# PinataFarms/DAD-3DHeads

Measured on AMD Instinct MI355X. Metric: images/sec (FLAME decode + 445-lmk projection), batch 64 @ 256^2, higher is better.
Workload: dtype f32

## Files before the change

### dad-3dheads_amd/csrc/capi.cpp

```cpp
#include <algorithm>
#include <cmath>
#include <cstdlib>
#include <cstring>
#include <memory>
#include <mutex>

#include "common.hpp"

namespace dad3d {

static thread_local std::string g_last_error;

void set_error(const char* fmt, ...) {
    char buf[1024];
    va_list ap;
    va_start(ap, fmt);
    vsnprintf(buf, sizeof buf, fmt, ap);
    va_end(ap);
    g_last_error = buf;
}

template <typename T>
static dad3d_status upload(T** dst, const std::vector<T>& src) {
    *dst = nullptr;
    const size_t bytes = std::max<size_t>(src.size(), 1) * sizeof(T);
    DAD3D_HIP_TRY(hipMalloc(reinterpret_cast<void**>(dst), bytes));
    if (!src.empty()) DAD3D_HIP_TRY(hipMemcpy(*dst, src.data(), src.size() * sizeof(T), hipMemcpyHostToDevice));
    return DAD3D_OK;
}

}

using namespace dad3d;

static void free_device(int device, std::initializer_list<void*> ptrs) {
    DeviceGuard guard(device);
    for (void* p : ptrs) (void)hipFree(p);
}

struct FlameConsts {
    int device = 0;
    float *d_bpack = nullptr, *d_jdirs = nullptr, *d_j0 = nullptr, *d_w8 = nullptr;
    float* d_bpack_pipe = nullptr;
    float split_b_scale = 1.0f;
    float* d_bpack_f16 = nullptr;
    std::mutex f16_mu;
    int n_tiles_pipe = 0;
    float* d_gpack = nullptr;
    std::mutex gpack_mutex;
    ~FlameConsts() { free_device(device, {d_bpack, d_jdirs, d_j0, d_w8, d_gpack, d_bpack_pipe, d_bpack_f16}); }
};

struct LandmarkList {
    int device = 0;
    int n = 0;
    int *d_head = nullptr, *d_next = nullptr;
    float4* d_vtab = nullptr;
    std::unique_ptr<FlameConsts> sub;
    int sub_verts = 0;
    float4* d_sub_vtab = nullptr;
    ~LandmarkList() { free_device(device, {d_head, d_next, d_vtab, d_sub_vtab}); }
};

struct FlameShape {
    int device = 0;
    int n_verts = 0, n_betas = 0;
    ParamLayout lay{};
    int parents[kNumJoints]{};
    int n_pose_feats = 0, pose_feat_first = 0;
    int kgroups = 0, ksteps = 0;
    int n_tiles = 0, n_tiles_pad8 = 0;
    int max_shape = 300;
    float image_size = 256.f;
};

struct dad3d_flame : FlameShape {
    std::shared_ptr<FlameConsts> c;
    std::shared_ptr<LandmarkList> lmk;
    int kernel_choice = -1;
    float* d_bwd_partials = nullptr;
    int bwd_cap = 0;
    float* d_grad_partials = nullptr;
    size_t grad_cap = 0;
    float* d_imgc = nullptr;
    unsigned* d_sync = nullptr;
    unsigned arrive_total = 0;
    int cap_nbb = 0;
    bool profiling = false;
    unsigned long long* d_trace = nullptr;
    uint64_t trace_capacity = 0;
    char* d_split_a = nullptr;
    int split_cap = 0;
    std::vector<char*> split_retired;
    hipEvent_t ev_first = nullptr, ev_last = nullptr;
    int prof_launches = 0;
    ~dad3d_flame() {
        DeviceGuard guard(device);
        for (void* p : {(void*)d_sync, (void*)d_imgc, (void*)d_bwd_partials, (void*)d_grad_partials, (void*)d_split_a}) (void)hipFree(p);
        for (char* p : split_retired) (void)hipFree(p);
        if (ev_first) (void)hipEventDestroy(ev_first);
        if (ev_last) (void)hipEventDestroy(ev_last);
    }
};

static int decode_kernel_choice() {
    static const int choice = [] {
        const char* e = getenv("DAD3D_DECODE_KERNEL");
        if (!e) return 0;
        if (e[0] == 'v' && e[1] == '1') return DAD3D_KERNEL_TWO_ROLE;
        if (std::strcmp(e, "split") == 0) return DAD3D_KERNEL_SPLIT_BF16;
        if (std::strcmp(e, "split_f16") == 0) return DAD3D_KERNEL_SPLIT_F16;
        return std::strcmp(e, "force_pipe") == 0 ? DAD3D_KERNEL_PIPELINED : DAD3D_KERNEL_AUTO;
    }();
    return choice;
}

static size_t frag_offset(int tile, int kgroups, int g, int col, int q) {
    return ((((size_t)tile * kgroups + g) * 4 + col / 16) * 64 + (col % 16) + 16 * q) * 4;
}
template <typename F>
static void for_each_fragment(std::vector<float>& pack, int n_tiles, int kgroups, F&& f) {
    for (int t = 0; t < n_tiles; ++t)
        for (int g = 0; g < kgroups; ++g)
            for (int col = 0; col < kTileCols; ++col)
                for (int q = 0; q < 4; ++q) f(t, g, col, q, &pack[frag_offset(t, kgroups, g, col, q)]);
}

static int grad_chunks(const dad3d_flame* h) { return (h->n_verts * 3 + kGradChunk - 1) / kGradChunk; }

static dad3d_status grad_inputs_prepare(dad3d_flame* h, int batch, hipStream_t s) {
    const int pad = (batch + kBlockImages - 1) / kBlockImages * kBlockImages;
    const int per_slice = grad_chunks_per_slice(pad);
    const size_t rows = (size_t)((grad_chunks(h) + per_slice - 1) / per_slice) * pad;
    bool need_pack;
    {
        std::lock_guard<std::mutex> lock(h->c->gpack_mutex);
        need_pack = h->c->d_gpack == nullptr;
    }
    const bool need_scratch = rows > h->grad_cap;
    if (!need_pack && !need_scratch) return DAD3D_OK;
    hipStreamCaptureStatus capture = hipStreamCaptureStatusNone;
    if (s != nullptr) (void)hipStreamIsCapturing(s, &capture);
    DAD3D_REQUIRE(capture == hipStreamCaptureStatusNone,
                  "the first training step of a handle (and the first at a larger batch) allocates: run it once before capturing a graph");
    DAD3D_REQUIRE(h->n_betas + 36 <= kGradRows, "dad3d_flame_grad_inputs: %d inputs exceed %d", h->n_betas + 36, kGradRows);
    if (need_pack) {
        std::lock_guard<std::mutex> lock(h->c->gpack_mutex);
        if (!h->c->d_gpack) {
            float* pack = nullptr;
            DAD3D_HIP_TRY(hipMalloc(reinterpret_cast<void**>(&pack), grad_pack_floats(grad_chunks(h)) * sizeof(float)));
            GradPackArgs pa{h->c->d_bpack, pack, h->kgroups, h->n_betas, h->n_pose_feats, h->pose_feat_first, h->n_betas + 36,
                            h->n_verts * 3, grad_chunks(h)};
            dad3d_status st = launch_grad_pack(pa, nullptr);
            if (st == DAD3D_OK && hipDeviceSynchronize() != hipSuccess) st = DAD3D_E_HIP;
            if (st) {
                (void)hipFree(pack);
                set_error("building the basis^T pack failed");
                return st;
            }
            h->c->d_gpack = pack;
        }
    }
    if (need_scratch) {
        DAD3D_HIP_TRY(hipDeviceSynchronize());
        (void)hipFree(h->d_grad_partials);
        h->d_grad_partials = nullptr;
        h->grad_cap = 0;
        DAD3D_HIP_TRY(hipMalloc(reinterpret_cast<void**>(&h->d_grad_partials), rows * kGradRows * sizeof(float)));
        h->grad_cap = rows;
    }
    return DAD3D_OK;
}

static dad3d_status flame_reserve(dad3d_flame* h, int nbb) {
    if (nbb <= h->cap_nbb) return DAD3D_OK;
    if (h->d_imgc) (void)hipFree(h->d_imgc);
    h->d_imgc = nullptr;
    h->cap_nbb = 0;
    DAD3D_HIP_TRY(hipMalloc(reinterpret_cast<void**>(&h->d_imgc), (size_t)nbb * kBlockImages * kImgConsts * sizeof(float)));
    h->cap_nbb = nbb;
    return DAD3D_OK;
}

static bool landmark_subset_enabled() {
    static const bool on = [] {
        const char* e = getenv("DAD3D_LANDMARK_SUBSET");
        return !(e && e[0] == '0');
    }();
    return on;
}

static dad3d_status build_landmark_sub(const dad3d_flame* h, const int64_t* idx, int n, const std::vector<float4>& vtab, LandmarkList* L) {
    std::vector<char> named(h->n_verts, 0);
    for (int s = 0; s < n; ++s) named[idx[s]] = 1;
    std::vector<int> uniq;
    for (int v = 0; v < h->n_verts; ++v)
        if (named[v]) uniq.push_back(v);
    const int nu = (int)uniq.size(), nt = (nu + kPipeTileVerts - 1) / kPipeTileVerts;
    if ((size_t)nu * 3 > (size_t)h->n_verts) return DAD3D_OK;
    std::vector<float> full((size_t)h->c->n_tiles_pipe * kPipeKGroups * 4 * 64 * 4), pack((size_t)nt * kPipeKGroups * 4 * 64 * 4, 0.0f);
    DAD3D_HIP_TRY(hipMemcpy(full.data(), h->c->d_bpack_pipe, full.size() * sizeof(float), hipMemcpyDeviceToHost));
    for_each_fragment(pack, nt, kPipeKGroups, [&](int t, int g, int col, int q, float* dst) {
        int src_tile = 0, src_col = col;
        if (col < 3 * kPipeTileVerts) {
            const int u = t * kPipeTileVerts + col / 3;
            if (u >= nu) return;
            src_tile = uniq[u] / kPipeTileVerts, src_col = (uniq[u] % kPipeTileVerts) * 3 + col % 3;
        }
        std::copy_n(&full[frag_offset(src_tile, kPipeKGroups, g, src_col, q)], 4, dst);
    });
    std::vector<float4> sub_vtab(nu);
    for (int u = 0; u < nu; ++u) sub_vtab[u] = vtab[uniq[u]];
    L->sub.reset(new FlameConsts);
    L->sub->device = h->device;
    L->sub->n_tiles_pipe = nt;
    L->sub->split_b_scale = h->c->split_b_scale;
    L->sub_verts = nu;
    const dad3d_status st = upload(&L->sub->d_bpack_pipe, pack);
    return st ? st : upload(&L->d_sub_vtab, sub_vtab);
}

static dad3d_status build_landmarks(const dad3d_flame* h, const int64_t* idx, int n, std::shared_ptr<LandmarkList>* out) {
    const int V = h->n_verts;
    std::vector<int> head(V, -1), next(n, -1);
    for (int s = n - 1; s >= 0; --s) {
        next[s] = head[idx[s]];
        head[idx[s]] = s;
    }
    std::vector<int> head2((size_t)V * 2, -1);
    for (int v = 0; v < V; ++v)
        if (head[v] >= 0) head2[(size_t)v * 2] = head[v], head2[(size_t)v * 2 + 1] = next[head[v]];
    auto L = std::make_shared<LandmarkList>();
    L->device = h->device;
    L->n = n;
    dad3d_status st;
    if ((st = upload(&L->d_head, head2)) || (st = upload(&L->d_next, next))) return st;
    if (h->c->d_bpack_pipe) {
        std::vector<float> w8((size_t)V * 8);
        DAD3D_HIP_TRY(hipMemcpy(w8.data(), h->c->d_w8, w8.size() * sizeof(float), hipMemcpyDeviceToHost));
        std::vector<float4> vtab(V);
        for (int v = 0; v < V; ++v) {
            const float* w = &w8[(size_t)v * 8];
            float fh, fn;
            memcpy(&fh, &head2[(size_t)v * 2], 4), memcpy(&fn, &head2[(size_t)v * 2 + 1], 4);
            vtab[v] = float4{w[5] + w[2], w[2], fh, fn};
        }
        if ((st = upload(&L->d_vtab, vtab))) return st;
        if (landmark_subset_enabled() && n > 0 && (st = build_landmark_sub(h, idx, n, vtab, L.get()))) return st;
    }
    *out = std::move(L);
    return DAD3D_OK;
}

extern "C" {

const char* dad3d_last_error(void) { return g_last_error.c_str(); }
void dad3d_clear_error(void) { g_last_error.clear(); }
int dad3d_version(void) { return DAD3D_VERSION; }
const char* dad3d_build_info(void) {
    static const std::string info = [] {
        int rt = 0, drv = 0;
        (void)hipRuntimeGetVersion(&rt);
        (void)hipDriverGetVersion(&drv);
        char buf[384];
        snprintf(buf, sizeof buf, "built: clang %s, HIP headers %d.%d.%d; running: HIP runtime %d, driver %d", __clang_version__, HIP_VERSION_MAJOR,
                 HIP_VERSION_MINOR, HIP_VERSION_PATCH, rt, drv);
        return std::string(buf);
// ... 153 lines not shown
    h->lmk = parent->lmk;
    h->kernel_choice = parent->kernel_choice;
    dad3d_status st;
    if ((st = upload(&h->d_sync, std::vector<unsigned>(kSyncWords, 0u))) || (st = flame_reserve(h.get(), 1))) return st;
    *out = h.release();
    return DAD3D_OK;
}

int dad3d_flame_num_params(const dad3d_flame* h) { return h ? h->lay.n_params : -1; }
int dad3d_flame_num_verts(const dad3d_flame* h) { return h ? h->n_verts : -1; }
int dad3d_flame_num_landmarks(const dad3d_flame* h) { return h ? h->lmk->n : -1; }
int dad3d_flame_num_landmark_vertices(const dad3d_flame* h) { return h ? h->lmk->sub_verts : 0; }

dad3d_status dad3d_flame_set_landmarks(dad3d_flame* h, const int64_t* idx, int n) {
    DAD3D_REQUIRE(h && n >= 0 && (idx || n == 0), "dad3d_flame_set_landmarks: bad argument");
    for (int s = 0; s < n; ++s)
        DAD3D_REQUIRE(idx[s] >= 0 && idx[s] < h->n_verts, "landmark index %lld out of range [0,%d)", (long long)idx[s], h->n_verts);
    DeviceGuard guard(h->device);
    std::shared_ptr<LandmarkList> list;
    dad3d_status st = build_landmarks(h, idx, n, &list);
    if (st) return st;
    DAD3D_HIP_TRY(hipDeviceSynchronize());
    h->lmk = std::move(list);
    return DAD3D_OK;
}

static uint64_t trace_entries_two_role(const dad3d_flame* h, int batch) {
    const uint64_t nbb = (batch + kBlockImages - 1) / kBlockImages, pose_blocks = ((uint64_t)(batch + 3) / 4 + 7) / 8 * 8;
    return ((uint64_t)h->n_tiles_pad8 * nbb * 8 + pose_blocks * 4) * 32;
}
static uint64_t trace_entries_pipe(const dad3d_flame* h) { return (uint64_t)h->c->n_tiles_pipe * 8 * 32; }

static dad3d_status ensure_basis_f16(FlameConsts* c, hipStream_t s) {
    std::lock_guard<std::mutex> lock(c->f16_mu);
    if (c->d_bpack_f16) return DAD3D_OK;
    hipStreamCaptureStatus capture = hipStreamCaptureStatusNone;
    if (s != nullptr) (void)hipStreamIsCapturing(s, &capture);
    DAD3D_REQUIRE(capture == hipStreamCaptureStatusNone, "the first fp16-split decode of a model builds its basis planes: run it once before capturing a graph");
    const size_t bytes = (size_t)c->n_tiles_pipe * kPipeKGroups * 4 * 64 * 4 * sizeof(float);
    float* d = nullptr;
    DAD3D_HIP_TRY(hipMalloc(reinterpret_cast<void**>(&d), bytes));
    dad3d_status st = launch_split_basis_f16(c->d_bpack_pipe, d, c->n_tiles_pipe, c->split_b_scale, s);
    if (st == DAD3D_OK && hipStreamSynchronize(s) != hipSuccess) {
        set_error("ensure_basis_f16: hipStreamSynchronize failed");
        st = DAD3D_E_HIP;
    }
    if (st) {
        (void)hipFree(d);
        return st;
    }
    c->d_bpack_f16 = d;
    return DAD3D_OK;
}

static dad3d_status ensure_split_scratch(dad3d_flame* h, int n_phase, hipStream_t s) {
    if (n_phase <= h->split_cap) return DAD3D_OK;
    hipStreamCaptureStatus capture = hipStreamCaptureStatusNone;
    if (s != nullptr) (void)hipStreamIsCapturing(s, &capture);
    DAD3D_REQUIRE(capture == hipStreamCaptureStatusNone,
                  "the first split-kernel decode of a handle (and the first at a larger batch) allocates: run it once before capturing a graph");
    if (h->d_split_a) h->split_retired.push_back(h->d_split_a);
    h->d_split_a = nullptr, h->split_cap = 0;
    DAD3D_HIP_TRY(hipMalloc(reinterpret_cast<void**>(&h->d_split_a), (size_t)n_phase * kSplitBlockBytes));
    DAD3D_HIP_TRY(hipMemsetAsync(h->d_split_a, 0, (size_t)n_phase * kSplitBlockBytes, s));
    h->split_cap = n_phase;
    return DAD3D_OK;
}

static int resolve_kernel(const dad3d_flame* h, int pinned, int batch, unsigned flags, bool posed) {
    const bool pipe_covers = h->c->d_bpack_pipe && !posed && !(flags & (DAD3D_COMPAT_CROSS_B3 | DAD3D_ZERO_ROTATION)) &&
                             (size_t)batch * h->n_verts * 12 < ((size_t)1 << 31) && (size_t)batch * std::max(h->lmk->n, 1) * 8 < ((size_t)1 << 31);
    if (pinned == DAD3D_KERNEL_TWO_ROLE || (pinned == DAD3D_KERNEL_AUTO && !pipe_covers)) return DAD3D_KERNEL_TWO_ROLE;
    if (pipe_covers) return pinned == DAD3D_KERNEL_AUTO ? DAD3D_KERNEL_PIPELINED : pinned;
    set_error("dad3d_flame_decode: the %s kernel does not cover this launch (model, flags or output size)",
              pinned == DAD3D_KERNEL_PIPELINED ? "pipelined" : "split");
    return -1;
}

static dad3d_status decode_impl(dad3d_flame* h, float* params, int batch, unsigned flags, float* verts3d, float* proj,
                                float* lmk_xy, int32_t* lmk_px, float* posed, void* stream) {
    DAD3D_REQUIRE(h, "dad3d_flame_decode: null handle");
    DAD3D_REQUIRE(batch >= 0, "dad3d_flame_decode: negative batch");
    if (batch == 0) return DAD3D_OK;
    DAD3D_REQUIRE(params, "dad3d_flame_decode: null params");
    DAD3D_REQUIRE(!((flags & DAD3D_FLIP_Z) && (flags & DAD3D_TO_2D)), "DAD3D_FLIP_Z needs a 3-component projection");
    DAD3D_REQUIRE(!(posed && (flags & DAD3D_COMPAT_CROSS_B3)), "DAD3D_COMPAT_CROSS_B3 is inference-only (dad3d_flame_decode_posed refuses it)");
    DeviceGuard guard(h->device);
    hipStream_t s = static_cast<hipStream_t>(stream);
    const int pinned = h->kernel_choice >= 0 ? h->kernel_choice : decode_kernel_choice();
    const int kernel = resolve_kernel(h, pinned, batch, flags, posed != nullptr);
    if (kernel < 0) return DAD3D_E_UNSUPPORTED;
    const LandmarkList& L = *h->lmk;
    const int n_lmk = (lmk_xy || lmk_px) ? L.n : 0;

    const bool on_sub = L.sub && !verts3d && !proj && n_lmk && !h->d_trace && pinned != DAD3D_KERNEL_PIPELINED;
    FlameConsts* c = on_sub ? L.sub.get() : h->c.get();
    const float4* vtab = on_sub ? L.d_sub_vtab : L.d_vtab;
    const int n_verts = on_sub ? L.sub_verts : h->n_verts;

    dad3d_status st;
    if (kernel == DAD3D_KERNEL_SPLIT_BF16 || kernel == DAD3D_KERNEL_SPLIT_F16) {
        DAD3D_REQUIRE(!h->d_trace, "dad3d_flame_decode: the split kernels have no trace stamps");
        const int n_phase = (batch + kSplitRows - 1) / kSplitRows;
        st = ensure_split_scratch(h, n_phase, s);
        if (!st && kernel == DAD3D_KERNEL_SPLIT_F16) st = ensure_basis_f16(c, s);
        if (!st && kernel == DAD3D_KERNEL_SPLIT_F16 && L.sub) st = ensure_basis_f16(L.sub.get(), s);
        if (st) return st;
        SplitArgs sa{};
        sa.params = params;
        sa.bpack = c->d_bpack_pipe;
        sa.bpack_f16 = c->d_bpack_f16;
        sa.vtab = vtab;
        sa.lmk_next = L.d_next;
        sa.verts3d = verts3d;
        sa.proj = proj;
        sa.lmk_xy = lmk_xy;
        sa.lmk_px = lmk_px;
        sa.aplanes = h->d_split_a;
        sa.b_scale = c->split_b_scale;
        sa.n_params = h->lay.n_params;
        sa.batch = batch;
        sa.n_phase = n_phase;
        sa.n_tiles = c->n_tiles_pipe;
        split_chunking(sa.n_tiles, n_phase, &sa.n_chunks, &sa.phases_per_chunk);
        sa.n_verts = n_verts;
        sa.n_lmk = n_lmk;
        sa.image_size = h->image_size;
        sa.flags = flags & 0xFFu;
        st = launch_flame_decode_split(sa, kernel, s);
    } else if (kernel == DAD3D_KERNEL_PIPELINED) {
        DAD3D_REQUIRE(!h->d_trace || h->trace_capacity >= trace_entries_pipe(h), "dad3d_flame_decode: the trace buffer holds %llu entries, "
                      "this launch stamps %llu (dad3d_flame_debug_trace_entries)", (unsigned long long)h->trace_capacity,
                      (unsigned long long)trace_entries_pipe(h));
        PipeArgs pa{};
        pa.params = params;
        pa.bpack = c->d_bpack_pipe;
        pa.vtab = vtab;
        pa.lmk_next = L.d_next;
        pa.verts3d = verts3d;
        pa.proj = proj;
        pa.lmk_xy = lmk_xy;
        pa.lmk_px = lmk_px;
        pa.trace = h->d_trace;
        pa.n_params = h->lay.n_params;
        pa.batch = batch;
        pa.n_half = (batch + kPipeHalf - 1) / kPipeHalf;
        pa.n_tiles = c->n_tiles_pipe;
        pa.n_verts = n_verts;
        pa.n_lmk = n_lmk;
        pa.image_size = h->image_size;
        pa.flags = flags & 0xFFu;
        pa.n_chunks = 1;
        if (!h->d_trace && (!proj || (flags & DAD3D_TO_2D))) pipe_chunking(pa.n_tiles, pa.n_half, &pa.chunk_half, &pa.n_chunks, &pa.wg_per_xcd);
        st = launch_flame_decode_pipe(pa, s);
    } else {
        DAD3D_REQUIRE(!h->d_trace || h->trace_capacity >= trace_entries_two_role(h, batch), "dad3d_flame_decode: the trace buffer holds %llu "
                      "entries, this launch stamps %llu (dad3d_flame_debug_trace_entries)", (unsigned long long)h->trace_capacity,
                      (unsigned long long)trace_entries_two_role(h, batch));
        if (posed && batch <= DAD3D_GRAD_INPUTS_MAX_BATCH && h->n_betas + 36 <= kGradRows && (st = grad_inputs_prepare(h, batch, s))) return st;
        const int nbb = (batch + kBlockImages - 1) / kBlockImages;
        if (nbb > h->cap_nbb) {
            DAD3D_HIP_TRY(hipDeviceSynchronize());
            if ((st = flame_reserve(h, nbb))) return st;
        }
        DecodeArgs da{};
        da.params = params;
        da.bpack = h->c->d_bpack;
        da.jdirs = h->c->d_jdirs;
        da.j0 = h->c->d_j0;
        da.weights8 = h->c->d_w8;
        da.lmk_head = L.d_head;
        da.lmk_next = L.d_next;
        da.imgc = h->d_imgc;
        da.sync = h->d_sync;
        da.verts3d = verts3d;
        da.proj = proj;
        da.lmk_xy = lmk_xy;
        da.lmk_px = lmk_px;
        da.posed = posed;
        da.trace = h->d_trace;
        da.lay = h->lay;
        std::copy(h->parents, h->parents + kNumJoints, da.parents);
        da.batch = batch;
        da.nbb = nbb;
        da.n_tiles = h->n_tiles;
        da.n_tiles_pad8 = h->n_tiles_pad8;
        da.n_verts = h->n_verts;
        da.n_lmk = n_lmk;
        da.n_pose_blocks = (batch + 3) / 4;
        da.n_pose_blocks_pad8 = (da.n_pose_blocks + 7) / 8 * 8;
        da.n_betas = h->n_betas;
        da.max_shape = h->max_shape;
        da.betas_contiguous = (h->lay.shape_n == 300 && h->lay.expr_n == 100 && h->lay.shape_off == 0 && h->lay.expr_off == 300);
        da.kgroups = h->kgroups;
        hipStreamCaptureStatus capture = hipStreamCaptureStatusNone;
        if (s != nullptr) (void)hipStreamIsCapturing(s, &capture);
        const bool device_epoch = capture != hipStreamCaptureStatusNone;
        da.arrive_target = h->arrive_total + (unsigned)da.n_pose_blocks;
        da.spin_limit = 1u << 20;
#ifdef DAD3D_DIAG_SPIN_ENV
        if (const char* e = getenv("DAD3D_SPIN_LIMIT")) da.spin_limit = (unsigned)atoi(e);
#endif
        da.image_size = h->image_size;
        da.flags = (flags & 0xFFu) | (device_epoch ? kDeviceEpoch : 0u);
        st = launch_flame_decode(da, s);
        if (!st && !device_epoch) h->arrive_total = da.arrive_target;
    }
    if (!st && h->profiling) ++h->prof_launches;
    return st;
}

dad3d_status dad3d_flame_decode(dad3d_flame* h, float* params, int batch, unsigned flags, float* verts3d, float* proj,
                                float* lmk_xy, int32_t* lmk_px, void* stream) {
    return decode_impl(h, params, batch, flags, verts3d, proj, lmk_xy, lmk_px, nullptr, stream);
}

dad3d_status dad3d_flame_decode_posed(dad3d_flame* h, float* params, int batch, unsigned flags, float* verts3d, float* proj,
                                      float* posed, void* stream) {
    return decode_impl(h, params, batch, flags, verts3d, proj, nullptr, nullptr, posed, stream);
}

dad3d_status dad3d_flame_decode_host(dad3d_flame* h, float* params, int batch, unsigned flags, float* verts3d,
                                     float* proj, float* lmk_xy, int32_t* lmk_px) {
    DAD3D_REQUIRE(h, "dad3d_flame_decode_host: null handle");
    DAD3D_REQUIRE(batch >= 0, "dad3d_flame_decode_host: negative batch");
    if (batch == 0) return DAD3D_OK;
    DAD3D_REQUIRE(params, "dad3d_flame_decode_host: null params");
    DeviceGuard guard(h->device);
    const size_t B = batch, V = h->n_verts, P = h->lay.n_params, NL = h->lmk->n;
    const size_t pc = (flags & DAD3D_TO_2D) ? 2 : 3;
    const size_t n_par = B * P, n_v = verts3d ? B * V * 3 : 0, n_p = proj ? B * V * pc : 0;
    const size_t n_lx = lmk_xy ? B * NL * 2 : 0, n_lp = lmk_px ? B * NL * 2 : 0;
    float* d = nullptr;
    DAD3D_HIP_TRY(hipMalloc(reinterpret_cast<void**>(&d), (n_par + n_v + n_p + n_lx + n_lp + 4) * sizeof(float)));
    float* d_par = d;
    float* d_v = n_v ? d_par + n_par : nullptr;
    float* d_p = n_p ? d_par + n_par + n_v : nullptr;
    float* d_lx = n_lx ? d_par + n_par + n_v + n_p : nullptr;
    int32_t* d_lp = n_lp ? reinterpret_cast<int32_t*>(d_par + n_par + n_v + n_p + n_lx) : nullptr;
    dad3d_status st = DAD3D_OK;
    auto fail = [&](hipError_t e, const char* what) {
        if (e != hipSuccess && st == DAD3D_OK) {
            set_error("%s failed: %s", what, hipGetErrorString(e));
            st = DAD3D_E_HIP;
        }
    };
    fail(hipMemcpy(d_par, params, n_par * sizeof(float), hipMemcpyHostToDevice), "hipMemcpy(params)");
    if (!st) st = dad3d_flame_decode(h, d_par, batch, flags, d_v, d_p, d_lx, d_lp, nullptr);
    if (!st) fail(hipDeviceSynchronize(), "hipDeviceSynchronize");
    if (!st && (flags & DAD3D_MUTATE_PARAMS)) fail(hipMemcpy(params, d_par, n_par * sizeof(float), hipMemcpyDeviceToHost), "hipMemcpy");
    if (!st && n_v) fail(hipMemcpy(verts3d, d_v, n_v * sizeof(float), hipMemcpyDeviceToHost), "hipMemcpy");
    if (!st && n_p) fail(hipMemcpy(proj, d_p, n_p * sizeof(float), hipMemcpyDeviceToHost), "hipMemcpy");
    if (!st && n_lx) fail(hipMemcpy(lmk_xy, d_lx, n_lx * sizeof(float), hipMemcpyDeviceToHost), "hipMemcpy");
    if (!st && n_lp) fail(hipMemcpy(lmk_px, d_lp, n_lp * sizeof(int32_t), hipMemcpyDeviceToHost), "hipMemcpy");
    (void)hipFree(d);
    return st;
}

dad3d_status dad3d_flame_readjust_params(dad3d_flame* h, float* params, int batch, const float* pads_scale,
                                         float pad_left, float pad_top, float scale, void* stream) {
    DAD3D_REQUIRE(h && batch >= 0, "dad3d_flame_readjust_params: bad argument");
    if (batch == 0) return DAD3D_OK;
    DAD3D_REQUIRE(params, "dad3d_flame_readjust_params: null params");
    DeviceGuard guard(h->device);
    return launch_readjust(params, batch, h->lay, pads_scale, pad_left, pad_top, scale, h->image_size,
                           static_cast<hipStream_t>(stream));
}

dad3d_status dad3d_flame_select_kernel(dad3d_flame* h, int which) {
    DAD3D_REQUIRE(h && which >= DAD3D_KERNEL_AUTO && which <= DAD3D_KERNEL_SPLIT_F16, "dad3d_flame_select_kernel: bad argument");
    h->kernel_choice = which;
    return DAD3D_OK;
}

dad3d_status dad3d_flame_handoff_timeouts(dad3d_flame* h, unsigned* count) {
    DAD3D_REQUIRE(h && count, "null argument");
    DeviceGuard guard(h->device);
    DAD3D_HIP_TRY(hipDeviceSynchronize());
    DAD3D_HIP_TRY(hipMemcpy(count, h->d_sync + 1, sizeof(unsigned), hipMemcpyDeviceToHost));
    return DAD3D_OK;
}

uint64_t dad3d_flame_debug_trace_entries(const dad3d_flame* h, int batch) {
    if (!h || batch <= 0) return 0;
    return std::max(trace_entries_two_role(h, batch), trace_entries_pipe(h));
}

dad3d_status dad3d_flame_debug_trace(dad3d_flame* h, unsigned long long* device_buffer, uint64_t capacity) {
    DAD3D_REQUIRE(h, "null handle");
    h->d_trace = device_buffer;
    h->trace_capacity = device_buffer ? capacity : 0;
    return DAD3D_OK;
}

dad3d_status dad3d_flame_decode_backward(dad3d_flame* h, int batch, unsigned flags, const float* consts, const float* posed,
                                         const float* grad_verts3d, const float* grad_proj, float* grad_posed,
                                         float* grad_consts, void* stream) {
    DAD3D_REQUIRE(h, "dad3d_flame_decode_backward: null handle");
    DAD3D_REQUIRE(batch >= 0, "dad3d_flame_decode_backward: negative batch");
    if (batch == 0) return DAD3D_OK;
    DAD3D_REQUIRE(consts && posed && grad_posed && grad_consts, "dad3d_flame_decode_backward: null argument");
    DAD3D_REQUIRE(grad_verts3d || grad_proj, "dad3d_flame_decode_backward: no upstream gradient");
    DAD3D_REQUIRE(!((flags & DAD3D_FLIP_Z) && (flags & DAD3D_TO_2D)), "DAD3D_FLIP_Z needs a 3-component projection");
    DAD3D_REQUIRE(!(posed && (flags & DAD3D_COMPAT_CROSS_B3)), "DAD3D_COMPAT_CROSS_B3 is inference-only (dad3d_flame_decode_posed refuses it)");
    DeviceGuard guard(h->device);
    BackwardArgs ba{};
    ba.weights8 = h->c->d_w8;
// ... 1709 lines not shown
```

### dad-3dheads_amd/csrc/common.hpp

```cpp
#pragma once

#include <hip/hip_runtime.h>

#include <atomic>
#include <cstdarg>
#include <cstdint>
#include <cstdio>
#include <string>
#include <vector>

#include "../../include/dad3d.h"

namespace dad3d {

void set_error(const char* fmt, ...);

#define DAD3D_HIP_TRY(expr)                                                                      \
    do {                                                                                         \
        hipError_t e__ = (expr);                                                                 \
        if (e__ != hipSuccess) {                                                                 \
            ::dad3d::set_error("%s failed: %s (%s:%d)", #expr, hipGetErrorString(e__), __FILE__, \
                               __LINE__);                                                        \
            return DAD3D_E_HIP;                                                                  \
        }                                                                                        \
    } while (0)

#define DAD3D_REQUIRE(cond, ...)            \
    do {                                    \
        if (!(cond)) {                      \
            ::dad3d::set_error(__VA_ARGS__); \
            return DAD3D_E_INVALID;         \
        }                                   \
    } while (0)

struct PerDeviceOnce {
    std::atomic<unsigned long long> mask[4] = {};
    static int current() {
        int d = 0;
        (void)hipGetDevice(&d);
        return d & 255;
    }
    bool done(int d) const { return (mask[d >> 6].load(std::memory_order_acquire) >> (d & 63)) & 1ull; }
    void set(int d) { mask[d >> 6].fetch_or(1ull << (d & 63), std::memory_order_release); }
};

struct DeviceGuard {
    int prev = -1;
    bool ok = true;
    explicit DeviceGuard(int device) {
        if (hipGetDevice(&prev) != hipSuccess) prev = -1;
        if (prev != device) ok = (hipSetDevice(device) == hipSuccess);
    }
    ~DeviceGuard() {
        if (prev >= 0) (void)hipSetDevice(prev);
    }
};

constexpr int kTileVerts = 21;
constexpr int kTileCols = 64;
constexpr int kBlockImages = 64;
constexpr int kImgConsts = 84;
constexpr int kNumJoints = 5;
constexpr int kOutStride = 68;
constexpr int kSyncWords = 1025;
constexpr unsigned kDeviceEpoch = 0x100u;

struct ParamLayout {
    int n_params;
    int shape_off, shape_n;
    int expr_off, expr_n;
    int jaw_off, jaw_n;
    int rot_off;
    int eye_off, eye_n;
    int neck_off, neck_n;
    int trans_off;
    int scale_off;
};

struct DecodeArgs {
    float* params;
    const float* bpack;
    const float* jdirs;
    const float* j0;
    const float* weights8;
    const int* lmk_head;
    const int* lmk_next;
    float* imgc;
    unsigned* sync;
    float* verts3d;
    float* proj;
    float* lmk_xy;
    int32_t* lmk_px;
    unsigned long long* trace;
    ParamLayout lay;
    int parents[kNumJoints];
    int batch, nbb, n_tiles, n_tiles_pad8, n_verts, n_lmk;
    int n_pose_blocks, n_pose_blocks_pad8;
    int n_betas, max_shape;
    int betas_contiguous;
    int kgroups;
    unsigned arrive_target;
    unsigned spin_limit;
    float image_size;
    unsigned flags;
    float* posed;
};

dad3d_status launch_flame_decode(const DecodeArgs& a, hipStream_t s);

constexpr int kPipeTileVerts = 20;
constexpr int kPipeHalf = 32;
constexpr int kPipeKGroups = 26;
struct PipeArgs {
    float* params;
    const float* bpack;
    const float4* vtab;
    const int* lmk_next;
    float* verts3d;
    float* proj;
    float* lmk_xy;
    int32_t* lmk_px;
    unsigned long long* trace;
    int n_params, batch, n_half, n_tiles, n_verts, n_lmk;
    float image_size;
    unsigned flags;
    int chunk_half, n_chunks, wg_per_xcd;
};
inline void pipe_chunking(int n_tiles, int n_half, int* chunk_half, int* n_chunks, int* wg_per_xcd) {
    *chunk_half = 0, *n_chunks = 1, *wg_per_xcd = 0;
    const int max_chunks = 256 / n_tiles;
    if (max_chunks < 2 || n_half < 2) return;
    *chunk_half = (n_half + max_chunks - 1) / max_chunks;
    *n_chunks = (n_half + *chunk_half - 1) / *chunk_half;
    *wg_per_xcd = (n_tiles * *n_chunks + 7) / 8;
}
struct PipeGeom {
    unsigned flags;
    int wg_per_xcd, n_chunks, n_tiles;
};
constexpr bool pipe_geom_fits(int wg_per_xcd, int n_chunks, int n_tiles) {
    return wg_per_xcd >= 0 && wg_per_xcd < 256 && n_chunks >= 1 && n_chunks <= 256 && n_tiles >= 0 && n_tiles < 256;
}
constexpr unsigned pipe_geom_word(unsigned flags, int wg_per_xcd, int n_chunks, int n_tiles) {
    return (flags & 0xFFu) | (unsigned)wg_per_xcd << 8 | (unsigned)(n_chunks - 1) << 16 | (unsigned)n_tiles << 24;
}
constexpr PipeGeom pipe_geom_unpack(unsigned w) {
    return PipeGeom{w & 0xFFu, (int)(w >> 8 & 0xFFu), (int)(w >> 16 & 0xFFu) + 1, (int)(w >> 24)};
}
dad3d_status launch_flame_decode_pipe(const PipeArgs& a, hipStream_t s);
size_t flame_decode_pipe_lds_bytes();

constexpr int kSplitRows = 16;
constexpr int kSplitKGroups = 13;
constexpr int kSplitRowBytes = 848;
constexpr int kSplitPlaneBytes = (3 * kSplitRows * kSplitRowBytes + 1023) / 1024 * 1024;
constexpr int kSplitConstBytes = (kSplitRows * 24 * 4 + 1023) / 1024 * 1024;
constexpr int kSplitBlockBytes = kSplitPlaneBytes + kSplitConstBytes;
struct SplitArgs {
    float* params;
    const float* bpack;
    const float* bpack_f16;
    const float4* vtab;
    const int* lmk_next;
    float* verts3d;
    float* proj;
    float* lmk_xy;
    int32_t* lmk_px;
    char* aplanes;
    float b_scale;
    int n_params, batch, n_phase, n_tiles, n_verts, n_lmk;
    int n_chunks, phases_per_chunk;
    float image_size;
    unsigned flags;
};
inline void split_chunking(int n_tiles, int n_phase, int* n_chunks, int* phases_per_chunk) {
    *n_chunks = 1, *phases_per_chunk = n_phase;
    const int max_chunks = 256 / n_tiles;
    if (max_chunks < 2 || n_phase < 2) return;
    *phases_per_chunk = (n_phase + max_chunks - 1) / max_chunks;
    *n_chunks = (n_phase + *phases_per_chunk - 1) / *phases_per_chunk;
}
dad3d_status launch_flame_decode_split(const SplitArgs& a, int form, hipStream_t s);
float split_basis_scale(float max_abs);
dad3d_status launch_split_basis_f16(const float* bpack, float* bpack_f16, int n_tiles, float scale, hipStream_t s);
size_t flame_decode_split_lds_bytes();

constexpr int kBackwardConsts = 72;
struct BackwardArgs {
    const float* weights8;
    const float* consts;
    const float* posed;
    const float* g_verts3d;
    const float* g_proj;
    float* g_posed;
    float* g_consts;
    float* partials;
    int batch, n_verts, nsplit;
    float image_size;
    unsigned flags;
};
dad3d_status launch_flame_backward(const BackwardArgs& a, hipStream_t s);
constexpr int kBackwardMaxSplit = 8;

constexpr int kGradChunk = 256;
constexpr int kGradQuarters = 4;
constexpr int kGradQuarterRows = 128;
constexpr int kGradRows = kGradQuarters * kGradQuarterRows;
struct GradPackArgs {
    const float* bpack;
    float* gpack;
    int kgroups, n_betas, n_pose_feats, pose_feat_first, n_inputs, n_cols, n_chunks;
};
struct GradInputsArgs {
    const float* g_posed;
    const float* gpack;
    float* partials;
    float* g_inputs;
    int batch, batch_pad, n_cols, n_chunks, n_inputs;
    int chunks_per_slice, n_slices;
};
inline int grad_chunks_per_slice(int batch_pad) { return batch_pad / kBlockImages >= 4 ? 4 : batch_pad / kBlockImages >= 2 ? 2 : 1; }
size_t grad_pack_floats(int n_chunks);
dad3d_status launch_grad_pack(const GradPackArgs& a, hipStream_t s);
dad3d_status launch_grad_inputs(const GradInputsArgs& a, hipStream_t s);

struct ChainArgs {
    const float* params;
    const float* jdirs;
    const float* j0;
    float* inputs;
    float* consts;
    const float* g_inputs;
    const float* g_consts;
    float* g_params;
    ParamLayout lay;
    int parents[kNumJoints];
    int batch, n_betas, max_shape;
};
dad3d_status launch_pose_chain(const ChainArgs& a, bool vjp, hipStream_t s);
dad3d_status launch_readjust(float* params, int batch, ParamLayout lay, const float* pads_scale, float pad_left,
                             float pad_top, float scale, float img_size, hipStream_t s);
size_t flame_decode_lds_bytes(int kgroups);

struct MeshDev {
    const int* tri;
    const int* adj_ptr;
    const int* adj_face;
    const int4* adj_tri;
    int ntri, nver;
};

constexpr int kNormalChunkings = 4;
struct NormalChunksDev {
    const uint2* faces;
    int face_ptr[9];
    const unsigned short* slot;
    const uint4* row8;
    int chunks, vpb, max_faces;
};

dad3d_status launch_tri_normal(const MeshDev& m, float* tri_normal, const float* vertices, int batch, int norm_flg,
                               hipStream_t s);
dad3d_status launch_ver_normal(const MeshDev& m, float* ver_normal, const float* tri_normal, int batch,
                               unsigned flags, hipStream_t s);
dad3d_status launch_get_normal(const MeshDev& m, const NormalChunksDev* nc, float* ver_normal, const float* vertices,
                               int batch, unsigned flags, hipStream_t s);
size_t normal_table_lds_bytes(int nver, int max_faces);
struct NormalPlan {
    int form, chunks, vpb;
    const NormalChunksDev* nc;
    size_t lds;
};
NormalPlan plan_get_normal(const MeshDev& m, const NormalChunksDev* nc, int batch);
NormalPlan plan_phong(const MeshDev& m, const NormalChunksDev* nc, bool normals_given, int batch);
NormalPlan plan_render_light(const MeshDev& m, const NormalChunksDev* nc, int h, int w);
size_t raster_scratch_bytes(const MeshDev& m, int batch, int h, int w);
dad3d_status raster_scratch_init(const MeshDev& m, void* scratch, int batch, int h, int w, hipStream_t s);
dad3d_status launch_rasterize(const MeshDev& m, const NormalChunksDev* nc, void* scratch, unsigned long long* trace, uint8_t* image, const float* vertices,
                              const float* colors, float* depth, int32_t* tri_buf, float* bary, int batch, int h,
                              int w, int c, int render_flags, int mode, const dad3d_light* light_cfg, hipStream_t s, float alpha = 1.0f);
dad3d_status launch_render_texture(const MeshDev& m, void* scratch, void* image, int image_u8, const float* vertices, const float4* tex_tri,
                                   const void* texture, int texture_u8, size_t tex_image_stride, float* depth, int batch, int h, int w, int c,
                                   int tex_h, int tex_w, int tex_c, int nearest, hipStream_t s);
dad3d_status launch_phong(const MeshDev& m, const NormalChunksDev* nc, float* light, const float* vertices, const float* normals,
                          float* normals_out, int batch, const dad3d_light& cfg, hipStream_t s);
dad3d_status frames_check_shapes(const char* who, const int64_t* frames_host, int n_frames, int* total_tiles);
size_t frames_scratch_bytes(int ntri, int n_frames, int n_heads, int total_tiles);
dad3d_status launch_rasterize_frames(const MeshDev& m, void* scratch, const int64_t* frames, int n_frames, int total_tiles, const float* vertices,
                                     const float* colors, const int32_t* image_index, int n_heads, int reverse, int32_t* flags, hipStream_t s);
dad3d_status launch_render_texture_frames(const MeshDev& m, void* scratch, const int64_t* frames, int n_frames, int total_tiles,
                                          const float* vertices, const float4* tex_tri, const void* texture, int texture_u8, size_t tex_head_stride,
                                          int tex_h, int tex_w, int tex_c, int nearest, const int32_t* image_index, int n_heads, int32_t* flags,
                                          hipStream_t s);

dad3d_status launch_project_vertices(const float* vertices, const float* model_view, const float* projection,
                                     const float* frame, int batch, int nver, float* world_homo, float* xy, int32_t* xy_int,
                                     hipStream_t s);

constexpr int kCubeStats = 28;
struct CubeLossArgs {
    const float* pred;
    const float* target;
    const int* region_ptr;
// ... 402 lines not shown
```

Baseline: 5.401 million.

## Add single-block head kernel for 33-64 row whole-mesh FLAME decode

Adds a specialised decode kernel used when the batch is between one and two pipe halves and no chunking is in effect. Each workgroup covers one vertex tile. Four producer waves stage the parameter rows into LDS, while four MFMA waves prefetch the basis deeply, compute the rotations and run the blend GEMM, with fine-grained LDS counters standing in for full barriers. The epilogue for the second row group is interleaved with its MFMA loop. This targets the latency of the generic pipelined kernel at batch 64, at the cost of a large new code path that can be turned off through an environment variable.

```diff
diff --git a/dad-3dheads_amd/csrc/capi.cpp b/dad-3dheads_amd/csrc/capi.cpp
--- a/dad-3dheads_amd/csrc/capi.cpp
+++ b/dad-3dheads_amd/csrc/capi.cpp
@@ -113,6 +113,13 @@
         return std::strcmp(e, "force_pipe") == 0 ? DAD3D_KERNEL_PIPELINED : DAD3D_KERNEL_AUTO;
     }();
     return choice;
+}
+static bool decode_halfblocks_forced() {
+    static const bool forced = [] {
+        const char* e = getenv("DAD3D_DECODE_KERNEL");
+        return e && std::strcmp(e, "halfblocks") == 0;
+    }();
+    return forced;
 }
 
 static size_t frag_offset(int tile, int kgroups, int g, int col, int q) {
@@ -572,7 +579,8 @@
         pa.flags = flags & 0xFFu;
         pa.n_chunks = 1;
         if (!h->d_trace && (!proj || (flags & DAD3D_TO_2D))) pipe_chunking(pa.n_tiles, pa.n_half, &pa.chunk_half, &pa.n_chunks, &pa.wg_per_xcd);
-        st = launch_flame_decode_pipe(pa, s);
+        const bool head = pa.chunk_half == 0 && batch > kPipeHalf && batch <= 2 * kPipeHalf && (verts3d || proj) && !decode_halfblocks_forced();
+        st = head ? launch_flame_decode_head(pa, s) : launch_flame_decode_pipe(pa, s);
     } else {
         DAD3D_REQUIRE(!h->d_trace || h->trace_capacity >= trace_entries_two_role(h, batch), "dad3d_flame_decode: the trace buffer holds %llu "
                       "entries, this launch stamps %llu (dad3d_flame_debug_trace_entries)", (unsigned long long)h->trace_capacity,
diff --git a/dad-3dheads_amd/csrc/common.hpp b/dad-3dheads_amd/csrc/common.hpp
--- a/dad-3dheads_amd/csrc/common.hpp
+++ b/dad-3dheads_amd/csrc/common.hpp
@@ -149,6 +149,7 @@
 }
 dad3d_status launch_flame_decode_pipe(const PipeArgs& a, hipStream_t s);
 size_t flame_decode_pipe_lds_bytes();
+dad3d_status launch_flame_decode_head(const PipeArgs& a, hipStream_t s);
 
 constexpr int kSplitRows = 16;
 constexpr int kSplitKGroups = 13;
diff --git a/dad-3dheads_amd/csrc/flame_decode_head.hip b/dad-3dheads_amd/csrc/flame_decode_head.hip
--- /dev/null
+++ b/dad-3dheads_amd/csrc/flame_decode_head.hip
@@ -0,0 +1,428 @@
+#pragma clang fp contract(off)
+#include "common.hpp"
+#include "flame_math.hpp"
+#include "flame_pipe_epilogue.hpp"
+
+#ifndef DAD3D_HEAD_DEPTH
+#define DAD3D_HEAD_DEPTH 6
+#endif
+#ifndef DAD3D_HEAD_R0_AT
+#define DAD3D_HEAD_R0_AT 1
+#endif
+
+namespace dad3d {
+
+namespace {
+
+using namespace pipe;
+
+constexpr int KG = kPipeKGroups;
+constexpr int TV = kPipeTileVerts;
+constexpr int kNumBeta = 400;
+constexpr int kJawCol = 3 * TV;
+constexpr int LD = 424;
+constexpr int OS = 76;
+constexpr int CS = 24;
+constexpr int kRows = 64;
+constexpr int kRows1 = 48;
+constexpr int kRound = 128;
+constexpr int D = DAD3D_HEAD_DEPTH < KG ? DAD3D_HEAD_DEPTH : KG;
+static_assert(D >= 6 && DAD3D_HEAD_R0_AT < D, "issue-ahead depth");
+struct Lds {
+    static constexpr int a_off = 0;
+    static constexpr int o_off = a_off + kRows * LD;
+    static constexpr int c_off = o_off + kRows * OS;
+    static constexpr int y_off = c_off + 2 * kRound * CS;
+    static constexpr int v_off = y_off + 4;
+    static constexpr int total = v_off + 4 * TV;
+    static_assert(total * 4 <= 160 * 1024, "LDS budget of one CU");
+};
+
+__device__ __forceinline__ int lds_peek(lds_int* p) { return __hip_atomic_load(p, __ATOMIC_RELAXED, __HIP_MEMORY_SCOPE_WORKGROUP); }
+__device__ __forceinline__ void wait_ge(lds_int* p, int target) {
+    while (lds_peek(p) < target) __builtin_amdgcn_s_sleep(1);
+    asm volatile("" ::: "memory");
+}
+__device__ __forceinline__ void wait_ge2(lds_int* p, int target, lds_int* q, int target_q) {
+    while ((int)(lds_peek(p) < target) | (int)(lds_peek(q) < target_q)) __builtin_amdgcn_s_sleep(1);
+    asm volatile("" ::: "memory");
+}
+__device__ __forceinline__ void arrive(lds_int* p, int lane) {
+    asm volatile("s_waitcnt lgkmcnt(0)" ::: "memory");
+    if (lane == 0) __hip_atomic_fetch_add(p, 1, __ATOMIC_RELAXED, __HIP_MEMORY_SCOPE_WORKGROUP);
+}
+__device__ __forceinline__ void phase_barrier() {
+    asm volatile("s_waitcnt lgkmcnt(0)\n\ts_barrier" ::: "memory");
+}
+
+}
+
+constexpr int kHeadPreloadDwords = 14;
+static_assert(4 * kHeadPreloadDwords == 4 * sizeof(void*) + 6 * sizeof(int), "the preloaded range ends with n_lmk");
+struct PipeLateArgs {
+    const int* lmk_next;
+    float *verts3d, *proj, *lmk_xy;
+    int32_t* lmk_px;
+    float image_size;
+};
+static_assert((4 * kHeadPreloadDwords) % alignof(PipeLateArgs) == 0, "`late` starts where the preloaded range ends: late_args() reads it there");
+template <bool TO2D>
+__global__ __launch_bounds__(512, 2) void flame_decode_head_kernel(float* params, const float* bpack, const float4* vtab, unsigned long long* trace_buf, int batch,
+                                                                   int n_verts, int n_params, int span_half, unsigned geom, int n_lmk, PipeLateArgs late) {
+    PipeArgs a;
+    a.params = params, a.bpack = bpack, a.vtab = vtab, a.trace = trace_buf, a.n_params = n_params, a.batch = batch, a.n_half = span_half, a.n_verts = n_verts, a.n_lmk = n_lmk;
+    a.flags = pipe_geom_unpack(geom).flags;
+    extern __shared__ __attribute__((aligned(16))) float smem[];
+    float* abuf = smem + Lds::a_off;
+    float* otile = smem + Lds::o_off;
+    float* cst = smem + Lds::c_off;
+    lds_int* parts = (lds_int*)(smem + Lds::y_off);
+
+    const int tid = threadIdx.x, lane = tid & 63, wave = tid >> 6;
+    const int tile = blockIdx.x, v0 = tile * TV;
+    const int B = a.batch, P = a.n_params;
+    const bool two = B > kRows1;
+    unsigned long long* trace = a.trace ? a.trace + ((size_t)tile * 8 + wave) * 32 : nullptr;
+    auto stamp = [&](int slot) {
+        if (trace && lane == 0) trace[slot] = __builtin_readcyclecounter();
+    };
+    if (trace && lane == 0) trace[12] = wall_clock64();
+    stamp(0);
+    if (tid < 4) __hip_atomic_store(parts + tid, 0, __ATOMIC_RELAXED, __HIP_MEMORY_SCOPE_WORKGROUP);
+    const unsigned nl = (unsigned)a.n_lmk;
+    EpiCtx cx;
+    __amdgpu_buffer_rsrc_t rs3, rsp;
+    unsigned outs = 0;
+    auto late_args = [&]() {
+        typedef const __attribute__((address_space(4))) char* kernarg_ptr;
+        typedef const __attribute__((address_space(4))) PipeLateArgs* late_ptr;
+        kernarg_ptr kp = (kernarg_ptr)__builtin_amdgcn_kernarg_segment_ptr();
+        asm volatile("" : "+s"(kp));
+        const late_ptr lp = reinterpret_cast<late_ptr>(kp + 4 * kHeadPreloadDwords);
+        a.lmk_next = lp->lmk_next, a.verts3d = lp->verts3d, a.proj = lp->proj, a.lmk_xy = lp->lmk_xy, a.lmk_px = lp->lmk_px, a.image_size = lp->image_size;
+        rs3 = __builtin_amdgcn_make_buffer_rsrc(reinterpret_cast<char*>(a.verts3d), 0, 0x7fffffff, 0x00020000);
+        rsp = __builtin_amdgcn_make_buffer_rsrc(reinterpret_cast<char*>(a.proj), 0, 0x7fffffff, 0x00020000);
+        cx.lx = reinterpret_cast<char*>(a.lmk_xy), cx.lp = reinterpret_cast<char*>(a.lmk_px);
+        outs = __builtin_amdgcn_readfirstlane((a.verts3d ? 1u : 0u) | (a.proj ? 2u : 0u));
+        asm volatile("" : "+s"(outs));
+        cx.lmk_next = a.lmk_next;
+        cx.image_size = a.image_size;
+    };
+    cx.zsign = (a.flags & DAD3D_FLIP_Z) ? -1.0f : 1.0f;
+    float4* const vt_lds = reinterpret_cast<float4*>(smem + Lds::v_off);
+    auto fin4 = [&](int row0, int w) {
+        const int fi = lane & 3, fu = lane >> 2, b = row0 + 4 * w + fi;
+        const float4* cp = reinterpret_cast<const float4*>(cst + b * CS);
+        const float4 c0 = cp[0], c1 = cp[1], c2 = cp[2], c3 = cp[3], c4 = cp[4], c5 = cp[5];
+        const float* ot = otile + b * OS;
+        const float jx = ot[kJawCol], jy = ot[kJawCol + 1], jz = ot[kJawCol + 2];
+        const unsigned vrow = (unsigned)b * (unsigned)a.n_verts + (unsigned)(v0 + fu), bnl = (unsigned)b * nl;
+        {
+            const float4 t = vt_lds[fu];
+            const bool live = b < B && v0 + fu < a.n_verts;
+            finish_vertex<TO2D, 0>(cx, rs3, rsp, c0, c1, c2, c3, c4, c5, jx, jy, jz, ot[3 * fu], ot[3 * fu + 1], ot[3 * fu + 2], t.x, t.y, __float_as_int(t.z), __float_as_int(t.w),
+                                   live && (outs & 1u), live && (outs & 2u), live && nl > 0 && __float_as_int(t.z) >= 0, vrow, bnl);
+        }
+        if (fu < TV - 16) {
+            const int j = fu + 16;
+            const float4 t = vt_lds[j];
+            const bool live = b < B && v0 + j < a.n_verts;
+            finish_vertex<TO2D, 16>(cx, rs3, rsp, c0, c1, c2, c3, c4, c5, jx, jy, jz, ot[3 * j], ot[3 * j + 1], ot[3 * j + 2], t.x, t.y, __float_as_int(t.z), __float_as_int(t.w),
+                                    live && (outs & 1u), live && (outs & 2u), live && nl > 0 && __float_as_int(t.z) >= 0, vrow, bnl);
+        }
+    };
+    auto fin2 = [&](int row0) {
+        const int fi = lane & 1, fu = min(lane >> 1, TV - 1), b = row0 + 2 * wave + fi;
+        const float4* cp = reinterpret_cast<const float4*>(cst + b * CS);
+        const float4 c0 = cp[0], c1 = cp[1], c2 = cp[2], c3 = cp[3], c4 = cp[4], c5 = cp[5];
+        const float* ot = otile + b * OS;
+        const float jx = ot[kJawCol], jy = ot[kJawCol + 1], jz = ot[kJawCol + 2];
+        const unsigned vrow = (unsigned)b * (unsigned)a.n_verts + (unsigned)(v0 + fu), bnl = (unsigned)b * nl;
+        const float4 t = vt_lds[fu];
+        const bool live = b < B && (lane >> 1) < TV && v0 + fu < a.n_verts;
+        finish_vertex<TO2D, 0>(cx, rs3, rsp, c0, c1, c2, c3, c4, c5, jx, jy, jz, ot[3 * fu], ot[3 * fu + 1], ot[3 * fu + 2], t.x, t.y, __float_as_int(t.z), __float_as_int(t.w),
+                               live && (outs & 1u), live && (outs & 2u), live && nl > 0 && __float_as_int(t.z) >= 0, vrow, bnl);
+    };
+
+    if (wave >= 4) {
+        const int fw = wave - 4;
+        const int lr = lane >> 5, lc = lane & 31;
+        float4 pre[19];
+        const float* prow[6];
+#pragma unroll
+        for (int jj = 0; jj < 6; ++jj) prow[jj] = a.params + (size_t)min(12 * fw + 2 * jj + lr, B - 1) * P + 4 * lc;
+        auto load_slab = [&](int sl) {
+#pragma unroll
+            for (int jj = 0; jj < 6; ++jj) {
+                const f4u v = *reinterpret_cast<const f4u*>(prow[jj] + 128 * sl);
+                pre[6 * sl + jj] = float4{v.x, v.y, v.z, v.w};
+                __builtin_amdgcn_sched_barrier(0);
+            }
+        };
+        auto write_slab = [&](int sl) {
+#pragma unroll
+            for (int jj = 0; jj < 6; ++jj) *reinterpret_cast<float4*>(abuf + (12 * fw + 2 * jj + lr) * LD + 128 * sl + 4 * lc) = pre[6 * sl + jj];
+        };
+        load_slab(0);
+        const float4 vt_row = a.vtab[min(v0 + min(lane, TV - 1), a.n_verts - 1)];
+        stamp(1);
+        phase_barrier();
+        stamp(6);
+        load_slab(1);
+        load_slab(2);
+        {
+            const int r = min(lane >> 2, 11);
+            const f4u v = *reinterpret_cast<const f4u*>(a.params + (size_t)min(12 * fw + r, B - 1) * P + 384 + 4 * (lane & 3));
+            pre[18] = float4{v.x, v.y, v.z, v.w};
+        }
+        late_args();
+        write_slab(0);
+        arrive(parts, lane);
+        stamp(7);
+        write_slab(1);
+        arrive(parts + 1, lane);
+        write_slab(2);
+        if (lane < 48) *reinterpret_cast<float4*>(abuf + (12 * fw + (lane >> 2)) * LD + 384 + 4 * (lane & 3)) = pre[18];
+        arrive(parts + 2, lane);
+        if (fw == 3 && lane < TV) vt_lds[lane] = vt_row;
+        stamp(2);
+        if (two) {
+            float4 q[7];
+            const float* qrow[2];
+#pragma unroll
+            for (int jj = 0; jj < 2; ++jj) qrow[jj] = a.params + (size_t)min(kRows1 + 4 * fw + 2 * jj + lr, B - 1) * P + 4 * lc;
+#pragma unroll
+            for (int sl = 0; sl < 3; ++sl)
+#pragma unroll
+                for (int jj = 0; jj < 2; ++jj) {
+                    const f4u v = *reinterpret_cast<const f4u*>(qrow[jj] + 128 * sl);
+                    q[2 * sl + jj] = float4{v.x, v.y, v.z, v.w};
+                }
+            {
+                const f4u v = *reinterpret_cast<const f4u*>(a.params + (size_t)min(kRows1 + 4 * fw + min(lane >> 2, 3), B - 1) * P + 384 + 4 * (lane & 3));
+                q[6] = float4{v.x, v.y, v.z, v.w};
+            }
+            stamp(16);
+#pragma unroll
+            for (int sl = 0; sl < 3; ++sl)
+#pragma unroll
+                for (int jj = 0; jj < 2; ++jj) *reinterpret_cast<float4*>(abuf + (kRows1 + 4 * fw + 2 * jj + lr) * LD + 128 * sl + 4 * lc) = q[2 * sl + jj];
+            if (lane < 16) *reinterpret_cast<float4*>(abuf + (kRows1 + 4 * fw + (lane >> 2)) * LD + 384 + 4 * (lane & 3)) = q[6];
+            stamp(17);
+        }
+        stamp(18);
+        phase_barrier();
+        stamp(19);
+        if (two) {
+            fin4(32, fw);
+            stamp(21);
+            phase_barrier();
+            stamp(23);
+            fin2(kRows1);
+        } else {
+            fin4(0, wave);
+            fin2(32);
+        }
+        stamp(5);
+        if (trace && lane == 0) trace[13] = wall_clock64();
+        return;
+    }
+
+    const float4* bsrc = reinterpret_cast<const float4*>(a.bpack) + ((size_t)tile * KG * 4 + wave) * 64 + lane;
+    f4u raw0 = {}, raw1 = {};
+    f3u raw2 = {};
+    float raw_scale = 0.f;
+    {
+        const float* prow = a.params + (size_t)min(32 * wave + (lane & 31), B - 1) * P + kNumBeta;
+        raw0 = *reinterpret_cast<const f4u*>(prow), raw1 = *reinterpret_cast<const f4u*>(prow + 4), raw2 = *reinterpret_cast<const f3u*>(prow + 8);
+        raw_scale = prow[12];
+    }
+    auto write_round = [&]() {
+        const float jaw[3] = {raw0.x, raw0.y, raw0.z};
+        const float rot6[6] = {raw0.w, raw1.x, raw1.y, raw1.z, raw1.w, raw2.x};
+        float Dm[9], G[9];
+        rodrigues_minus_identity_lean(jaw, Dm);
+        rot6_to_matrix_lean(rot6, G);
+        const float sp1 = raw_scale + 1.0f;
+        const float s = sp1 < 1e-8f ? 1e-8f : sp1;
+        if (wave < 2 && lane < 32) {
+            float4* tail = reinterpret_cast<float4*>(abuf + (32 * wave + lane) * LD + kNumBeta);
+            tail[0] = float4{Dm[0], Dm[1], Dm[2], Dm[3]};
+            tail[1] = float4{Dm[4], Dm[5], Dm[6], Dm[7]};
+            tail[2] = float4{Dm[8], 1.0f, 0.f, 0.f};
+            tail[3] = float4{0.f, 0.f, 0.f, 0.f};
+        }
+        if (lane < 32) {
+            float4* c = reinterpret_cast<float4*>(cst + (32 * wave + lane) * CS);
+            c[0] = float4{Dm[0], Dm[1], Dm[2], Dm[3]};
+            c[1] = float4{Dm[4], Dm[5], Dm[6], Dm[7]};
+            c[2] = float4{Dm[8], G[0], G[1], G[2]};
+            c[3] = float4{G[3], G[4], G[5], G[6]};
+            c[4] = float4{G[7], G[8], s, raw2.y};
+            c[5] = float4{raw2.z, 0.f, 0.f, 0.f};
+            const int b = 32 * wave + lane;
+            if ((a.flags & DAD3D_MUTATE_PARAMS) && tile == 0 && b < B)
+                store_tz(a.params + ((unsigned)b * (unsigned)P + (unsigned)(kNumBeta + 11)));
+        }
+    };
+    float4 bq[KG];
+    const float* afrag0 = abuf + (lane & 15) * LD + 4 * (lane >> 4);
+    float* const ot0 = otile + ((lane >> 4) * 4) * OS + wave * 16 + (lane & 15);
+
+    late_args();
+    stamp(6);
+    phase_barrier();
+    stamp(7);
+#pragma unroll
+    for (int G = 0; G < D; ++G) {
+        bq[G] = bsrc[(size_t)G * 256];
+        __builtin_amdgcn_sched_barrier(0);
+        if (G == DAD3D_HEAD_R0_AT) {
+            write_round();
+            if (wave < 2) arrive(parts + 2, lane);
+            arrive(parts + 3, lane);
+            stamp(4);
+            __builtin_amdgcn_sched_barrier(0);
+        }
+    }
+    {
+        f32x4 acc[3] = {f32x4{0.f, 0.f, 0.f, 0.f}, f32x4{0.f, 0.f, 0.f, 0.f}, f32x4{0.f, 0.f, 0.f, 0.f}};
+        float4 af[3], an[3] = {};
+        stamp(16);
+        wait_ge(parts, 4);
+#pragma unroll
+        for (int m = 0; m < 3; ++m) af[m] = *reinterpret_cast<const float4*>(afrag0 + m * 16 * LD);
+#pragma unroll
+        for (int G = 0; G < KG; ++G) {
+            if (G + D < KG) bq[G + D] = bsrc[(size_t)(G + D) * 256];
+            if (G + 1 == 8) wait_ge(parts + 1, 4);
+            if (G + 1 == 16) wait_ge2(parts + 2, 6, parts + 3, 4);
+            if (G + 1 < KG) {
+#pragma unroll
+                for (int m = 0; m < 3; ++m) an[m] = *reinterpret_cast<const float4*>(afrag0 + m * 16 * LD + 16 * (G + 1));
+            }
+            __builtin_amdgcn_sched_barrier(0);
+            if (G == 0) stamp(8);
+#pragma unroll
+            for (int s = 0; s < 4; ++s) {
+                const float bv = s == 0 ? bq[G].x : s == 1 ? bq[G].y : s == 2 ? bq[G].z : bq[G].w;
+#pragma unroll
+                for (int m = 0; m < 3; ++m) {
+                    const float av = s == 0 ? af[m].x : s == 1 ? af[m].y : s == 2 ? af[m].z : af[m].w;
+                    acc[m] = __builtin_amdgcn_mfma_f32_16x16x4f32(av, bv, acc[m], 0, 0, 0);
+                }
+            }
+            __builtin_amdgcn_sched_barrier(0);
+#pragma unroll
+            for (int m = 0; m < 3; ++m) af[m] = an[m];
+        }
+        stamp(2);
+#pragma unroll
+        for (int m = 0; m < 3; ++m)
+#pragma unroll
+            for (int q = 0; q < 4; ++q) ot0[(m * 16 + q) * OS] = acc[m][q];
+        stamp(17);
+    }
+    if (!two) {
+        phase_barrier();
+        stamp(18);
+        stamp(3);
+        fin4(0, wave);
+        fin2(32);
+        stamp(5);
+        if (trace && lane == 0) trace[13] = wall_clock64();
+        return;
+    }
+    const int ei = lane & 7, eu = lane >> 3, li = 8 * wave + ei;
+    float4 k0, k1, k2, k3, k4, k5;
+    {
+        const float4* c = reinterpret_cast<const float4*>(cst + li * CS);
+        k0 = c[0], k1 = c[1], k2 = c[2], k3 = c[3], k4 = c[4], k5 = c[5];
+    }
+    phase_barrier();
+    stamp(18);
+    float vW[3], vw2[3];
+    int lh[3], ln[3];
+    bool vl[3];
+#pragma unroll
+    for (int k = 0; k < 3; ++k) {
+        const float4 t = vt_lds[min(eu + 8 * k, TV - 1)];
+        vW[k] = t.x, vw2[k] = t.y, lh[k] = __float_as_int(t.z), ln[k] = __float_as_int(t.w);
+        vl[k] = eu + 8 * k < TV && v0 + eu + 8 * k < a.n_verts;
+    }
+    float jx = 0.f, jy = 0.f, jz = 0.f, ex = 0.f, ey = 0.f, ez = 0.f;
+    const float* const ot_e = otile + li * OS;
+    const unsigned e_vrow = (unsigned)li * (unsigned)a.n_verts + (unsigned)(v0 + eu), e_bnl = (unsigned)li * nl;
+    bool live3[3], livep[3], livel[3];
+#pragma unroll
+    for (int k = 0; k < 3; ++k) live3[k] = vl[k] && (outs & 1u), livep[k] = vl[k] && (outs & 2u), livel[k] = vl[k] && nl > 0 && lh[k] >= 0;
+    auto epi_fetch = [&](int k) {
+        const int j = eu + 8 * k;
+        ex = ot_e[3 * j], ey = ot_e[3 * j + 1], ez = ot_e[3 * j + 2];
+    };
+    auto epi_finish = [&](int k) {
+        if (k == 0) finish_vertex<TO2D, 0>(cx, rs3, rsp, k0, k1, k2, k3, k4, k5, jx, jy, jz, ex, ey, ez, vW[0], vw2[0], lh[0], ln[0], live3[0], livep[0], livel[0], e_vrow, e_bnl);
+        if (k == 1) finish_vertex<TO2D, 8>(cx, rs3, rsp, k0, k1, k2, k3, k4, k5, jx, jy, jz, ex, ey, ez, vW[1], vw2[1], lh[1], ln[1], live3[1], livep[1], livel[1], e_vrow, e_bnl);
+        if (k == 2) finish_vertex<TO2D, 16>(cx, rs3, rsp, k0, k1, k2, k3, k4, k5, jx, jy, jz, ex, ey, ez, vW[2], vw2[2], lh[2], ln[2], live3[2], livep[2], livel[2], e_vrow, e_bnl);
+    };
+    {
+        f32x4 acc = f32x4{0.f, 0.f, 0.f, 0.f};
+        const float* afrag = afrag0 + kRows1 * LD;
+        float4 af = *reinterpret_cast<const float4*>(afrag), an = {};
+        stamp(20);
+#pragma unroll
+        for (int G = 0; G < KG; ++G) {
+            if (G + 1 < KG) an = *reinterpret_cast<const float4*>(afrag + 16 * (G + 1));
+            __builtin_amdgcn_sched_barrier(0);
+            acc = __builtin_amdgcn_mfma_f32_16x16x4f32(af.x, bq[G].x, acc, 0, 0, 0);
+            acc = __builtin_amdgcn_mfma_f32_16x16x4f32(af.y, bq[G].y, acc, 0, 0, 0);
+            acc = __builtin_amdgcn_mfma_f32_16x16x4f32(af.z, bq[G].z, acc, 0, 0, 0);
+            acc = __builtin_amdgcn_mfma_f32_16x16x4f32(af.w, bq[G].w, acc, 0, 0, 0);
+            __builtin_amdgcn_sched_barrier(0);
+            af = an;
+            if (G == 0) {
+                jx = ot_e[kJawCol], jy = ot_e[kJawCol + 1], jz = ot_e[kJawCol + 2];
+                epi_fetch(0);
+            }
+            if (G == 3) epi_finish(0), epi_fetch(1);
+            if (G == 11) epi_finish(1), epi_fetch(2);
+            if (G == 19) epi_finish(2);
+            __builtin_amdgcn_sched_barrier(0);
+        }
+#pragma unroll
+        for (int q = 0; q < 4; ++q) ot0[(kRows1 + q) * OS] = acc[q];
+        stamp(21);
+    }
+    phase_barrier();
+    stamp(22);
+    stamp(3);
+    fin2(kRows1);
+    stamp(5);
+    if (trace && lane == 0) trace[13] = wall_clock64();
+}
+
+dad3d_status launch_flame_decode_head(const PipeArgs& a, hipStream_t s) {
+    static PerDeviceOnce attr_done;
+    const int dev = PerDeviceOnce::current();
+    const size_t lds = (size_t)Lds::total * sizeof(float);
+    DAD3D_REQUIRE(a.batch > kPipeHalf && a.batch <= kRows && a.chunk_half == 0 && (a.verts3d || a.proj),
+                  "launch_flame_decode_head: a whole-mesh launch of 33..64 rows with a vertex output, not %d rows", a.batch);
+    if (!attr_done.done(dev)) {
+        for (const void* k : {reinterpret_cast<const void*>(&flame_decode_head_kernel<true>), reinterpret_cast<const void*>(&flame_decode_head_kernel<false>)})
+            DAD3D_HIP_TRY(hipFuncSetAttribute(k, hipFuncAttributeMaxDynamicSharedMemorySize, (int)lds));
+        attr_done.set(dev);
+    }
+    const bool to2d = (a.flags & DAD3D_TO_2D) || !a.proj;
+    const unsigned geom = pipe_geom_word(a.flags, 0, 1, 0);
+    const PipeLateArgs late{a.lmk_next, a.verts3d, a.proj, a.lmk_xy, a.lmk_px, a.image_size};
+    if (to2d)
+        hipLaunchKernelGGL((flame_decode_head_kernel<true>), dim3(a.n_tiles), dim3(512), lds, s, a.params, a.bpack, a.vtab, a.trace, a.batch, a.n_verts, a.n_params, a.n_half, geom,
+                           a.n_lmk, late);
+    else
+        hipLaunchKernelGGL((flame_decode_head_kernel<false>), dim3(a.n_tiles), dim3(512), lds, s, a.params, a.bpack, a.vtab, a.trace, a.batch, a.n_verts, a.n_params, a.n_half, geom,
+                           a.n_lmk, late);
+    DAD3D_HIP_TRY(hipGetLastError());
+    return DAD3D_OK;
+}
+
+}
```

After: 5.798 million (median of 6 runs). 1.07x the previous value.
